# wangtong627/COR

Measured on AMD Instinct MI355X. Metric: query triplets/sec (forward + similarity + top-k), higher is better.
Workload: dtype bf16

## Files before the change

cor_amd/csrc/flash_attn.hip:

```cpp
#include <cstdlib>
#include <type_traits>

#include "common.h"

typedef short s16x4 __attribute__((ext_vector_type(4)));

namespace {

struct FlashArgs {
  const bf16_t* q; const bf16_t* k; const bf16_t* v; void* o;
  long q_sb, q_st, k_sb, k_st, v_sb, v_st, o_sb, o_st;
  int H, Tq, Tk;
  float scale_log2;
  float tbl_scale;
  const bf16_t* pad_row; const float* rel_h; const float* rel_w;
  int grid, S, nW, d3;
  int nqt;
  int rev;
};

constexpr int KT = 64;
constexpr int TILE_B = KT * 128;
constexpr int KV_BYTES = 4 * TILE_B;
constexpr int AUX_PER_WAVE = 8192;
constexpr float LOG2E = 1.4426950408889634f;

__device__ __forceinline__ int acc_row(int e, int h) { return (e & 3) + 8 * (e >> 2) + 4 * h; }

__device__ __forceinline__ float other_half(float x) {
  const unsigned u = __float_as_uint(x);
  const auto r = __builtin_amdgcn_permlane32_swap(u, u, false, false);
  return __uint_as_float((threadIdx.x & 32) ? r[0] : r[1]);
}

typedef float f32x2_t __attribute__((ext_vector_type(2)));
typedef __bf16 bf16x2_t __attribute__((ext_vector_type(2)));
__device__ __forceinline__ uint32_t pk2(float a, float b) {
  const f32x2_t v = {a, b};
  return __builtin_bit_cast(uint32_t, __builtin_convertvector(v, bf16x2_t));
}
__device__ __forceinline__ uint4 pack8(float f0, float f1, float f2, float f3, float f4, float f5, float f6, float f7) {
  uint4 u;
  u.x = pk2(f0, f1); u.y = pk2(f2, f3); u.z = pk2(f4, f5); u.w = pk2(f6, f7);
  return u;
}

__device__ __forceinline__ float sum2_bf16(uint32_t pair, float acc) {
  return __builtin_amdgcn_fdot2_f32_bf16(__builtin_bit_cast(bf16x2_t, pair), __builtin_bit_cast(bf16x2_t, 0x3f803f80u), acc, false);
}
__device__ __forceinline__ float max3f_(float a, float b, float c) { return fmaxf(fmaxf(a, b), c); }

__device__ __forceinline__ uint4 table_frag(const float* tbl, int j, int c, int h) {
  const float* p = tbl + (long)j * 64 + 16 * c + 8 * h;
  const f32x4 a = *(const f32x4*)p, b = *(const f32x4*)(p + 4);
  return pack8(a[0], a[1], a[2], a[3], b[0], b[1], b[2], b[3]);
}

template <typename TO, int HD, typename OFF>
__device__ __forceinline__ void store_o_rows(const f32x16 (&o)[(HD + 31) / 32], float inv, char* stg, TO* out, int lane, OFF&& off) {
  constexpr int DB = (HD + 31) / 32;
  const int r = lane & 31, h = lane >> 5;
  if constexpr (sizeof(TO) == 2) {
    constexpr int SR = HD * 2 + 16, NCHO = HD * 2 / 16;
#pragma unroll
    for (int db = 0; db < DB; ++db)
#pragma unroll
      for (int g = 0; g < 4; ++g) {
        if (db * 32 + 8 * g + 8 <= HD) {
          uint2 u;
          u.x = pk2(o[db][4 * g] * inv, o[db][4 * g + 1] * inv); u.y = pk2(o[db][4 * g + 2] * inv, o[db][4 * g + 3] * inv);
          *(uint2*)(stg + r * SR + (db * 32 + 8 * g + 4 * h) * 2) = u;
        }
      }
    __builtin_amdgcn_fence(__ATOMIC_ACQ_REL, "wavefront");
#pragma unroll
    for (int i = 0; i < (32 * NCHO + 63) / 64; ++i) {
      const int idx = lane + 64 * i, j = idx / NCHO, ch = idx - j * NCHO;
      if (idx < 32 * NCHO) {
        const uint4 v = *(const uint4*)(stg + j * SR + ch * 16);
        const long e = off(j);
        if (e >= 0) *(uint4*)(out + e + ch * 8) = v;
      }
    }
  } else {
#pragma unroll
    for (int db = 0; db < DB; ++db) {
#pragma unroll
      for (int g = 0; g < 4; ++g) {
        if (db * 32 + 8 * g + 8 <= HD) {
          const f32x4 v4 = {o[db][4 * g] * inv, o[db][4 * g + 1] * inv, o[db][4 * g + 2] * inv, o[db][4 * g + 3] * inv};
          *(f32x4*)(stg + r * 144 + (8 * g + 4 * h) * 4) = v4;
        }
      }
      __builtin_amdgcn_fence(__ATOMIC_ACQ_REL, "wavefront");
#pragma unroll
      for (int i = 0; i < 4; ++i) {
        const int j = (lane >> 3) + 8 * i, ch = lane & 7;
        const f32x4 v = *(const f32x4*)(stg + j * 144 + ch * 16);
        const long e = off(j);
        if (e >= 0 && db * 32 + 4 * ch + 4 <= HD) *(f32x4*)(out + e + db * 32 + ch * 4) = v;
      }
      __builtin_amdgcn_fence(__ATOMIC_ACQ_REL, "wavefront");
    }
  }
}

template <int HD>
__device__ __forceinline__ uint4 table_frag_hd(const float* tbl, int j, int c, int h) {
  if (16 * c + 8 * h + 8 > HD) return make_uint4(0, 0, 0, 0);
  const float* p = tbl + (long)j * HD + 16 * c + 8 * h;
  const f32x4 a = *(const f32x4*)p, b = *(const f32x4*)(p + 4);
  return pack8(a[0], a[1], a[2], a[3], b[0], b[1], b[2], b[3]);
}

template <int MODE, typename TO, int HD = 64>
__global__ void __launch_bounds__(256, 2) flash_fwd(const FlashArgs a) {
  extern __shared__ __attribute__((aligned(16))) char smem[];
  constexpr int KS = (HD + 15) / 16, DB = (HD + 31) / 32, NCH = HD * 2 / 16, NCHP = 2 * KS;
  constexpr int ROWB = HD == 64 ? 128 : 208, TILEB = KT * ROWB, KVB = 4 * TILEB;
  constexpr int NP = (KT * NCHP + 255) / 256;
  const int tid = threadIdx.x, lane = tid & 63, wave = tid >> 6;
  const int r = lane & 31, h = lane >> 5;
  const int wi0_ = xcd_remap(blockIdx.x, gridDim.x);
  const int wi_ = a.rev ? (int)gridDim.x - 1 - wi0_ : wi0_;
  const int qt_ = wi_ % a.nqt, hb_ = wi_ / a.nqt;
  const int head = hb_ % a.H, bz = hb_ / a.H;
  const int S = a.S;

  int b = bz, wy = 0, wx = 0;
  if (MODE == 2) { const int nw2 = a.nW * a.nW; b = bz / nw2; const int wi = bz - b * nw2; wy = wi / a.nW; wx = wi - wy * a.nW; }
  const int g2 = a.grid * a.grid;

  auto kv_src = [&](int kidx, const bf16_t*& kp, const bf16_t*& vp) {
    if (MODE == 0) {
      kp = a.k + bz * a.k_sb + (long)kidx * a.k_st + head * HD;
      vp = a.v + bz * a.v_sb + (long)kidx * a.v_st + head * HD;
    } else {
      long row; bool ok = true;
      if (MODE == 1) row = (long)b * g2 + kidx;
      else {
        const int ky = kidx / S, kx = kidx - ky * S, y = wy * S + ky, x = wx * S + kx;
        ok = y < a.grid && x < a.grid;
        row = (long)b * g2 + (long)y * a.grid + x;
      }
      const bf16_t* base = ok ? a.q + row * a.d3 : a.pad_row;
      kp = base + a.H * HD + head * HD;
      vp = base + 2 * a.H * HD + head * HD;
    }
  };

  int tq = qt_ * 128 + wave * 32 + r;
  bool qvalid = tq < a.Tq;
  tq = min(tq, a.Tq - 1);
  const int qh = MODE == 0 ? 0 : tq / S, qw = MODE == 0 ? 0 : tq - (tq / S) * S;
  const bf16_t* qp;
  long orow = 0;
  if (MODE == 0) qp = a.q + bz * a.q_sb + (long)tq * a.q_st + head * HD;
  else if (MODE == 1) { orow = (long)b * g2 + tq; qp = a.q + orow * a.d3 + head * HD; }
  else {
    const int y = wy * S + qh, x = wx * S + qw;
    const bool ok = y < a.grid && x < a.grid;
    qvalid = qvalid && ok;
    orow = (long)b * g2 + (long)min(y, a.grid - 1) * a.grid + min(x, a.grid - 1);
    qp = ok ? a.q + orow * a.d3 + head * HD : a.pad_row + head * HD;
  }
  uint4 qf[KS];
#pragma unroll
  for (int c = 0; c < KS; ++c) qf[c] = (16 * c + 8 * h + 8 <= HD) ? *(const uint4*)(qp + 16 * c + 8 * h) : make_uint4(0, 0, 0, 0);

  constexpr int TSTRIDE = MODE == 2 ? 56 : KT;
  int st_row[NP], st_ch[NP], st_k[NP], st_v[NP];
// ... 720 lines not shown
    if (t + 3 < nt) vsrc += tile_bytes;
    if (!(DBG & 1) && (DBG & 512)) { dma_tile(kd, vk0p, vk1p, ksrc_t); dma_tile(vd, vv0p, vv1p, vsrc_t); }
    const char *Vs = Vring + ((t + 3) & 3) * TILE_B, *Ks = Kring + ((t + 1) & 3) * TILE_B;
    const float rh0 = aux[t * 64 + r], rh1 = aux[t * 64 + 32 + r];
    u32x4 vf[8], kf[8];
    if (DBG & 4) { Vs = Vring; Ks = Kring; }
#pragma unroll
    for (int i = 0; i < 8; ++i) {
      const int kb = i >> 2, ks = (i >> 1) & 1, db = i & 1;
      if ((DBG & 4) && t > 0) { vf[i] = u32x4{(unsigned)t, (unsigned)i, 3u, 4u}; continue; }
      const char* vb = Vs + (kb * 32 + ks * 16) * 128 + v_trd[db];
      const s16x4 v0 = __builtin_amdgcn_ds_read_tr16_b64_v4i16((__attribute__((address_space(3))) s16x4*)(vb));
      const s16x4 v1 = __builtin_amdgcn_ds_read_tr16_b64_v4i16((__attribute__((address_space(3))) s16x4*)(vb + 8 * 128));
      vf[i] = __builtin_bit_cast(u32x4, __builtin_shufflevector(v0, v1, 0, 1, 2, 3, 4, 5, 6, 7));
    }
#pragma unroll
    for (int i = 0; i < 8; ++i) {
      if ((DBG & 4) && t > 0) { kf[i] = u32x4{(unsigned)t, (unsigned)i, 1u, 2u}; continue; }
      kf[i] = *(const u32x4*)(Ks + (i >> 2) * 32 * 128 + kch[i & 3]);
    }
    __builtin_amdgcn_sched_barrier(0);

    auto pv = [&](int n) __attribute__((always_inline)) {
      const int qb = n >> 3, kb = (n >> 2) & 1, ks = (n >> 1) & 1, db = n & 1;
      if (DBG & 32) { asm volatile("" : "+a"(o[qb][db]) : "a"(vf[kb * 4 + ks * 2 + db]), "v"(pf[qb][kb][ks])); return; }
      asm volatile("v_mfma_f32_32x32x16_bf16 %0, %1, %2, %0" : "+a"(o[qb][db]) : "a"(vf[kb * 4 + ks * 2 + db]), "v"(pf[qb][kb][ks]));
    };
    auto qk = [&](int g, int c) __attribute__((always_inline)) {
      const int qb = g >> 1, kb = g & 1;
      if (DBG & 64) { asm volatile("" : "+v"(s[qb][kb]) : "a"(kf[kb * 4 + c]), "a"(qf[qb][c]), "v"(wreg[qb][kb])); return; }
      if (c == 0) asm volatile("v_mfma_f32_32x32x16_bf16 %0, %1, %2, %3" : "=&v"(s[qb][kb]) : "a"(kf[kb * 4 + c]), "a"(qf[qb][c]), "v"(wreg[qb][kb]));
      else asm volatile("v_mfma_f32_32x32x16_bf16 %0, %1, %2, %0" : "+v"(s[qb][kb]) : "a"(kf[kb * 4 + c]), "a"(qf[qb][c]));
    };
    float mloc[2];
#pragma unroll
    for (int qb = 0; qb < 2; ++qb) {
      float m4[4];
#pragma unroll
      for (int kb = 0; kb < 2; ++kb)
#pragma unroll
        for (int g = 0; g < 2; ++g) {
          const int e = 8 * g;
          const f32x16& x = s[qb][kb];
          if (DBG & 16) { m4[kb * 2 + g] = x[e]; continue; }
          const float t0 = max3f_(x[e], x[e + 1], x[e + 2]), t1 = max3f_(x[e + 3], x[e + 4], x[e + 5]);
          m4[kb * 2 + g] = max3f_(max3f_(t0, t1, x[e + 6]), x[e + 7], -INFINITY);
        }
      mloc[qb] = fmaxf(max3f_(m4[0], m4[1], m4[2]), m4[3]);
      __builtin_amdgcn_sched_barrier(0);
      pv(qb);
    }
    float msub[2], al0 = 1.f, al1 = 1.f;
    bool resc;
    {
      const float ml0 = fmaxf(mloc[0], other_half(mloc[0])) + rh0, ml1 = fmaxf(mloc[1], other_half(mloc[1])) + rh1;
      resc = __builtin_amdgcn_ballot_w64(ml0 > m[0] + 8.0f || ml1 > m[1] + 8.0f) != 0;
      if (resc) {
        const float mn0 = fmaxf(m[0], ml0), mn1 = fmaxf(m[1], ml1);
        al0 = __builtin_amdgcn_exp2f(m[0] - mn0); al1 = __builtin_amdgcn_exp2f(m[1] - mn1);
        m[0] = mn0; m[1] = mn1;
        lsum[0][0] *= al0; lsum[0][1] *= al0; lsum[1][0] *= al1; lsum[1][1] *= al1;
      }
      msub[0] = m[0] - rh0; msub[1] = m[1] - rh1;
    }
    __builtin_amdgcn_sched_barrier(0);
    float pe[4] = {0.f, 0.f, 0.f, 0.f};
#pragma unroll
    for (int c = 0; c <= 16; ++c) {
      float pn[4];
      uint32_t d0 = 0, d1 = 0;
      const int cp = c - 1, gp = cp >> 2, qbp = gp >> 1, kbp = gp & 1, k4 = cp & 3;
      if (c < 16) {
        const int g = c >> 2, qb = g >> 1, kb = g & 1, e0 = 4 * (c & 3);
#pragma unroll
        for (int i = 0; i < 2; ++i) pn[i] = (DBG & 8) ? s[qb][kb][e0 + i] - msub[qb] : (DBG & 256) ? __builtin_amdgcn_exp2f(s[qb][kb][e0 + i]) : __builtin_amdgcn_exp2f(s[qb][kb][e0 + i] - msub[qb]);
      }
      if (c > 0) { d0 = pk2(pe[0], pe[1]); if (!(DBG & 128)) lsum[qbp][k4 & 1] = sum2_bf16(d0, lsum[qbp][k4 & 1]); else if (c == 1) lsum[qbp][k4 & 1] += __uint_as_float(d0); }
      if (!(DBG & 1) && !(DBG & 512)) {
        if (c == 2) dma_tile(kd, vk0p, vk1p, ksrc_t);
        if (c == 10) dma_tile(vd, vv0p, vv1p, vsrc_t);
      }
      if (c < 4) pv(2 + 2 * c);
      else if (c < 8) pv(6 + c);
      else if (c < 10) pv(6 + c);
      else if (c < 12) qk(1, c - 8);
      else if (c < 16) qk(2, c - 12);
      __builtin_amdgcn_sched_barrier(0);
      if (c < 16) {
        const int g = c >> 2, qb = g >> 1, kb = g & 1, e0 = 4 * (c & 3);
#pragma unroll
        for (int i = 2; i < 4; ++i) pn[i] = (DBG & 8) ? s[qb][kb][e0 + i] - msub[qb] : (DBG & 256) ? __builtin_amdgcn_exp2f(s[qb][kb][e0 + i]) : __builtin_amdgcn_exp2f(s[qb][kb][e0 + i] - msub[qb]);
      }
      if (c > 0) {
        d1 = pk2(pe[2], pe[3]); if (!(DBG & 128)) lsum[qbp][k4 & 1] = sum2_bf16(d1, lsum[qbp][k4 & 1]);
        u32x4& dst = pf[qbp][kbp][k4 >> 1];
        if (k4 & 1) { dst[2] = d0; dst[3] = d1; } else { dst[0] = d0; dst[1] = d1; }
      }
      if (c < 4) pv(3 + 2 * c);
      else if (c < 8) qk(0, c - 4);
      else if (c < 10) qk(1, c - 8);
      else if (c == 16) { qk(3, 0); qk(3, 1); qk(3, 2); qk(3, 3); }
#pragma unroll
      for (int i = 0; i < 4; ++i) pe[i] = pn[i];
      __builtin_amdgcn_sched_barrier(0);
    }
    asm volatile("" :: "v"(lsum[0][0]), "v"(lsum[0][1]), "v"(lsum[1][0]), "v"(lsum[1][1]));
    if (resc) {
#pragma unroll
      for (int db = 0; db < 2; ++db)
#pragma unroll
        for (int e = 0; e < 16; ++e) {
          float x0 = o[0][db][e], x1 = o[1][db][e], t0, t1;
          asm volatile("v_accvgpr_read_b32 %2, %0\n\tv_accvgpr_read_b32 %3, %1\n\tv_mul_f32 %2, %2, %4\n\tv_mul_f32 %3, %3, %5\n\t"
                       "v_accvgpr_write_b32 %0, %2\n\tv_accvgpr_write_b32 %1, %3"
                       : "+a"(x0), "+a"(x1), "=&v"(t0), "=&v"(t1) : "v"(al0), "v"(al1));
          o[0][db][e] = x0; o[1][db][e] = x1;
        }
    }
    if (!(DBG & 2)) {
      asm volatile("s_waitcnt vmcnt(6)" ::: "memory");
      __syncthreads();
    }
  }
  {
    asm volatile("s_waitcnt vmcnt(0)" ::: "memory");
    const char* Vs = Vring + ((nt - 1) & 3) * TILE_B;
#pragma unroll
    for (int kb = 0; kb < 2; ++kb)
#pragma unroll
      for (int ks = 0; ks < 2; ++ks)
#pragma unroll
        for (int db = 0; db < 2; ++db) {
          const char* vb = Vs + (kb * 32 + ks * 16) * 128 + v_trd[db];
          const s16x4 v0 = __builtin_amdgcn_ds_read_tr16_b64_v4i16((__attribute__((address_space(3))) s16x4*)(vb));
          const s16x4 v1 = __builtin_amdgcn_ds_read_tr16_b64_v4i16((__attribute__((address_space(3))) s16x4*)(vb + 8 * 128));
          const u32x4 vfr = __builtin_bit_cast(u32x4, __builtin_shufflevector(v0, v1, 0, 1, 2, 3, 4, 5, 6, 7));
#pragma unroll
          for (int qb = 0; qb < 2; ++qb)
            asm volatile("v_mfma_f32_32x32x16_bf16 %0, %1, %2, %0" : "+a"(o[qb][db]) : "a"(vfr), "v"(pf[qb][kb][ks]));
        }
    asm volatile("s_nop 7\n\ts_nop 7\n\ts_nop 7\n\ts_nop 7" ::: "memory");
  }
#pragma unroll
  for (int qb = 0; qb < 2; ++qb) {
    const float l = lsum[qb][0] + lsum[qb][1];
    const float inv = 1.0f / (l + other_half(l));
    auto off = [&](int j) -> long { return ((long)b * g2 + qh * S + qb * 32 + j) * (long)(a.H * 64) + head * 64; };
    store_o_rows<TO, 64>(o[qb], inv, (char*)aux, (TO*)a.o, lane, off);
    __builtin_amdgcn_fence(__ATOMIC_ACQ_REL, "wavefront");
  }
}

constexpr int WIN_ROWS = 224, WIN_KV = WIN_ROWS * 128, WIN_T = 27 * 32 * 4, WIN_LDS = 2 * WIN_KV + 7 * WIN_T;

template <typename TO>
__global__ void __launch_bounds__(448, 4) win_attn(const FlashArgs a) {
  extern __shared__ __attribute__((aligned(16))) char smem[];
  const int tid = threadIdx.x, lane = tid & 63, wave = __builtin_amdgcn_readfirstlane(tid >> 6);
  const int r = lane & 31, h = lane >> 5;
  const int bid = a.rev ? (int)gridDim.x - 1 - (int)blockIdx.x : (int)blockIdx.x;
  const int head = bid % a.H, win = bid / a.H;
  const int nw2 = a.nW * a.nW, b = win / nw2, wi = win - b * nw2, wy = wi / a.nW, wx = wi - wy * a.nW;
  const int g2 = a.grid * a.grid;
  char* Kt = smem; char* Vt = smem + WIN_KV;
  float* T = (float*)(smem + 2 * WIN_KV + wave * WIN_T);

  {
    const unsigned lds0 = __builtin_amdgcn_readfirstlane((unsigned)(size_t)((__attribute__((address_space(3))) char*)smem));
    const int sl = lane & 7;
    long colp[2]; bool okx[2];
#pragma unroll
    for (int hf = 0; hf < 2; ++hf) {
      const int kw = min(8 * hf + (lane >> 3), 13), x = wx * 14 + kw;
      okx[hf] = x < a.grid;
      colp[hf] = ((long)b * g2 + x) * a.d3 + head * 64;
    }
#pragma unroll
    for (int i8 = 0; i8 < 8; ++i8) {
      const int i = wave * 8 + i8;
      const bool isv = i >= 28;
      const int ii = isv ? i - 28 : i, kh = ii >> 1, hf = ii & 1, y = wy * 14 + kh;
      const int chunk = isv ? (sl ^ (((lane >> 4) & 1) << 2)) : (sl ^ (4 * hf + (lane >> 4)));
      const long plane = (long)(isv ? 2 : 1) * a.H * 64 + chunk * 8;
      const bf16_t* src = (y < a.grid && okx[hf]) ? a.q + colp[hf] + (long)y * a.grid * a.d3 + plane : a.pad_row + head * 64 + plane;
      glds16(src, lds0 + (isv ? WIN_KV : 0) + ii * 1024);
    }
  }

  const int tq = min(wave * 32 + r, 195);
  const int qh = (tq * 4682) >> 16, qw = tq - 14 * qh;
  uint4 qf[4];
  {
    const int y = wy * 14 + qh, x = wx * 14 + qw;
    const bf16_t* qp = (y < a.grid && x < a.grid) ? a.q + ((long)b * g2 + (long)y * a.grid + x) * a.d3 + head * 64 : a.pad_row + head * 64;
#pragma unroll
    for (int c = 0; c < 4; ++c) qf[c] = *(const uint4*)(qp + 16 * c + 8 * h);
  }

  float colb[8];
  uint4 tf[2][4];
#pragma unroll
  for (int tbl = 0; tbl < 2; ++tbl)
#pragma unroll
    for (int c = 0; c < 4; ++c) tf[tbl][c] = table_frag(tbl == 0 ? a.rel_w : a.rel_h, min(r, 26), c, h);
#pragma unroll
  for (int tbl = 0; tbl < 2; ++tbl) {
    f32x16 acc;
#pragma unroll
    for (int e = 0; e < 16; ++e) acc[e] = 0.f;
#pragma unroll
    for (int c = 0; c < 4; ++c)
      acc = __builtin_amdgcn_mfma_f32_32x32x16_bf16(__builtin_bit_cast(bf16x8, tf[tbl][c]), __builtin_bit_cast(bf16x8, qf[c]), acc, 0, 0, 0);
#pragma unroll
    for (int e = 0; e < 16; ++e) {
      const int row = acc_row(e, h);
      if (row < 27) T[row * 32 + r] = acc[e] * a.tbl_scale;
    }
    __builtin_amdgcn_fence(__ATOMIC_ACQ_REL, "wavefront");
    if (tbl == 0) {
#pragma unroll
      for (int e8 = 0; e8 < 8; ++e8) {
        const int kw = (e8 & 3) + 8 * (e8 >> 2) + 4 * h;
        colb[e8] = kw < 14 ? T[(qw - min(kw, 13) + 13) * 32 + r] : -INFINITY;
      }
      __builtin_amdgcn_fence(__ATOMIC_ACQ_REL, "wavefront");
    }
  }

  if (a.scale_log2 != 1.0f) {
#pragma unroll
    for (int c = 0; c < 4; ++c) {
      uint32_t w[4] = {qf[c].x, qf[c].y, qf[c].z, qf[c].w};
#pragma unroll
      for (int i = 0; i < 4; ++i) w[i] = pk2(__uint_as_float(w[i] << 16) * a.scale_log2, __uint_as_float(w[i] & 0xffff0000u) * a.scale_log2);
      qf[c] = make_uint4(w[0], w[1], w[2], w[3]);
    }
  }

  asm volatile("s_waitcnt vmcnt(0)" ::: "memory");
  __syncthreads();

  const int sw = (r >> 1) & 7;
  const int k_rd = r * 128, v_tr = (4 * h + ((lane & 15) >> 2)) * 128 + (16 * ((lane >> 4) & 1) + 4 * (lane & 3)) * 2;
  const int v_trd[2] = {v_tr + ((lane >> 3) & 1) * 64, v_tr + (1 - ((lane >> 3) & 1)) * 64};
  const int t_rd = (qh + 13) * 32 + r;
  f32x16 o[2], lsum;
#pragma unroll
  for (int e = 0; e < 16; ++e) { o[0][e] = 0.f; o[1][e] = 0.f; lsum[e] = 0.f; }
  float m = 0.f;
  const uint4 ones = make_uint4(0x3F803F80u, 0x3F803F80u, 0x3F803F80u, 0x3F803F80u);
#pragma unroll
  for (int blk = 0; blk < 7; ++blk) {
    const char* Kb = Kt + blk * 32 * 128 + k_rd;
    uint4 kf[4];
#pragma unroll
    for (int c = 0; c < 4; ++c) kf[c] = *(const uint4*)(Kb + (((2 * c + h) ^ sw) << 4));
    const float rm0 = T[t_rd - 32 * (2 * blk)] - m, rm1 = T[t_rd - 32 * (2 * blk + 1)] - m;
    f32x16 s;
#pragma unroll
    for (int e = 0; e < 16; ++e) s[e] = colb[e & 7] + (e < 8 ? rm0 : rm1);
#pragma unroll
    for (int c = 0; c < 4; ++c)
      s = __builtin_amdgcn_mfma_f32_32x32x16_bf16(__builtin_bit_cast(bf16x8, kf[c]), __builtin_bit_cast(bf16x8, qf[c]), s, 0, 0, 0);
    float mloc = max3f_(max3f_(s[0], s[1], s[2]), max3f_(s[3], s[4], s[5]), max3f_(s[6], s[7], s[8]));
    mloc = fmaxf(max3f_(mloc, max3f_(s[9], s[10], s[11]), max3f_(s[12], s[13], s[14])), s[15]);
    mloc = fmaxf(mloc, other_half(mloc));
    if (blk == 0 || __builtin_amdgcn_ballot_w64(mloc > 8.0f) != 0) {
      const float d = blk == 0 ? mloc : fmaxf(mloc, 0.f);
      const float alpha = __builtin_amdgcn_exp2f(-d);
      m += d;
#pragma unroll
      for (int e = 0; e < 16; ++e) s[e] -= d;
      if (blk != 0) {
        lsum[1] *= alpha; lsum[2] *= alpha;
#pragma unroll
        for (int e = 0; e < 16; ++e) { o[0][e] *= alpha; o[1][e] *= alpha; }
      }
    }
    uint4 pf[2];
    {
      f32x16 p;
#pragma unroll
      for (int e = 0; e < 16; ++e) p[e] = __builtin_amdgcn_exp2f(s[e]);
      pf[0] = pack8(p[0], p[1], p[2], p[3], p[4], p[5], p[6], p[7]);
      pf[1] = pack8(p[8], p[9], p[10], p[11], p[12], p[13], p[14], p[15]);
      lsum[1] = sum2_bf16(pf[0].y, sum2_bf16(pf[0].x, lsum[1])); lsum[2] = sum2_bf16(pf[0].w, sum2_bf16(pf[0].z, lsum[2]));
      lsum[1] = sum2_bf16(pf[1].y, sum2_bf16(pf[1].x, lsum[1])); lsum[2] = sum2_bf16(pf[1].w, sum2_bf16(pf[1].z, lsum[2]));
    }
#pragma unroll
    for (int ks = 0; ks < 2; ++ks) {
#pragma unroll
      for (int db = 0; db < 2; ++db) {
        const char* vb = Vt + (blk * 32 + ks * 16) * 128 + v_trd[db];
        const s16x4 v0 = __builtin_amdgcn_ds_read_tr16_b64_v4i16((__attribute__((address_space(3))) s16x4*)(vb));
        const s16x4 v1 = __builtin_amdgcn_ds_read_tr16_b64_v4i16((__attribute__((address_space(3))) s16x4*)(vb + 8 * 128));
        const uint2 u0 = __builtin_bit_cast(uint2, v0), u1 = __builtin_bit_cast(uint2, v1);
        const uint4 vfr = make_uint4(u0.x, u0.y, u1.x, u1.y);
        o[db] = __builtin_amdgcn_mfma_f32_32x32x16_bf16(__builtin_bit_cast(bf16x8, vfr), __builtin_bit_cast(bf16x8, pf[ks]), o[db], 0, 0, 0);
      }
    }
  }

  const float lhalf = lsum[1] + lsum[2];
  const float inv = 1.0f / (lhalf + other_half(lhalf));
  char* stg = (char*)T;
  TO* out = (TO*)a.o;
  auto off = [&](int jq) -> long {
    const int tj = wave * 32 + jq;
    if (tj >= 196) return -1;
    const int jh = (tj * 4682) >> 16, y = wy * 14 + jh, x = wx * 14 + (tj - 14 * jh);
    if (y >= a.grid || x >= a.grid) return -1;
    return ((long)b * g2 + (long)y * a.grid + x) * (long)(a.H * 64) + head * 64;
  };
  const long e0 = off(lane >> 2), e1 = off((lane >> 2) + 16);
  const int rd0 = (lane >> 2) * 80 + (lane & 3) * 16;
  __builtin_amdgcn_fence(__ATOMIC_ACQ_REL, "wavefront");
  if constexpr (sizeof(TO) == 2) {
#pragma unroll
    for (int db = 0; db < 2; ++db) {
#pragma unroll
      for (int g = 0; g < 4; ++g) {
        uint2 u;
        u.x = pk2(o[db][4 * g] * inv, o[db][4 * g + 1] * inv); u.y = pk2(o[db][4 * g + 2] * inv, o[db][4 * g + 3] * inv);
        *(uint2*)(stg + r * 80 + (8 * g + 4 * h) * 2) = u;
      }
      __builtin_amdgcn_fence(__ATOMIC_ACQ_REL, "wavefront");
      const uint4 v0 = *(const uint4*)(stg + rd0), v1 = *(const uint4*)(stg + rd0 + 16 * 80);
      if (e0 >= 0) *(uint4*)(out + e0 + db * 32 + (lane & 3) * 8) = v0;
      if (e1 >= 0) *(uint4*)(out + e1 + db * 32 + (lane & 3) * 8) = v1;
      __builtin_amdgcn_fence(__ATOMIC_ACQ_REL, "wavefront");
    }
  } else {
#pragma unroll
    for (int qd = 0; qd < 4; ++qd) {
      const int db = qd >> 1, g0 = 2 * (qd & 1);
#pragma unroll
      for (int gg = 0; gg < 2; ++gg) {
        const int g = g0 + gg;
        const f32x4 v4 = {o[db][4 * g] * inv, o[db][4 * g + 1] * inv, o[db][4 * g + 2] * inv, o[db][4 * g + 3] * inv};
        *(f32x4*)(stg + r * 80 + (8 * gg + 4 * h) * 4) = v4;
      }
      __builtin_amdgcn_fence(__ATOMIC_ACQ_REL, "wavefront");
      const f32x4 v0 = *(const f32x4*)(stg + rd0), v1 = *(const f32x4*)(stg + rd0 + 16 * 80);
      if (e0 >= 0) *(f32x4*)(out + e0 + qd * 16 + (lane & 3) * 4) = v0;
      if (e1 >= 0) *(f32x4*)(out + e1 + qd * 16 + (lane & 3) * 4) = v1;
      __builtin_amdgcn_fence(__ATOMIC_ACQ_REL, "wavefront");
    }
  }
}

template <typename TO>
int launch_win(const FlashArgs& a, int nwin, hipStream_t s) {
  static DevOnce once;
  cor_max_dyn_lds((const void*)win_attn<TO>, WIN_LDS, once);
  hipLaunchKernelGGL((win_attn<TO>), dim3(nwin * a.H), dim3(448), WIN_LDS, s, a);
  COR_CHECK_LAUNCH();
  return 0;
}

template <typename TO, bool STAMP = false, bool CB = false>
int launch_global_pipe(const FlashArgs& a, int nb, hipStream_t s) {
  const size_t lds = 6 * TILE_B + 4 * AUX_PER_WAVE;
  static DevOnce once;
  cor_max_dyn_lds((const void*)flash_global_pipe<TO, STAMP, CB>, (int)lds, once);
  FlashArgs b = a;
  b.nqt = cdiv(a.Tq, 128);
  hipLaunchKernelGGL((flash_global_pipe<TO, STAMP, CB>), dim3(b.nqt * a.H * nb), dim3(256), lds, s, b);
  COR_CHECK_LAUNCH();
  return 0;
}

template <typename TO, int DBG = 0>
int launch_global_w64(const FlashArgs& a, int nb, hipStream_t s) {
  const size_t lds = 8 * TILE_B + 4 * 64 * 64 * 4;
  static DevOnce once;
  cor_max_dyn_lds((const void*)flash_global_w64<TO, DBG>, (int)lds, once);
  FlashArgs b = a;
  b.nqt = a.Tq / 256;
  hipLaunchKernelGGL((flash_global_w64<TO, DBG>), dim3(b.nqt * a.H * nb), dim3(256), lds, s, b);
  COR_CHECK_LAUNCH();
  return 0;
}

template <int MODE, typename TO, int HD = 64>
int launch(const FlashArgs& a, int nb, hipStream_t s) {
  constexpr int ROWB = HD == 64 ? 128 : 208;
  const size_t lds = 4 * KT * ROWB + (MODE == 0 ? 0 : 4 * AUX_PER_WAVE);
  static DevOnce once;
  cor_max_dyn_lds((const void*)flash_fwd<MODE, TO, HD>, (int)lds, once);
  FlashArgs b = a;
  b.nqt = cdiv(a.Tq, 128);
  hipLaunchKernelGGL((flash_fwd<MODE, TO, HD>), dim3(b.nqt * a.H * nb), dim3(256), lds, s, b);
  COR_CHECK_LAUNCH();
  return 0;
}
template <int MODE, int HD>
int launch_t(const FlashArgs& a, int nb, int out_dtype, hipStream_t s) {
  if (out_dtype == COR_BF16) return launch<MODE, bf16_t, HD>(a, nb, s);
  if (out_dtype == COR_F32) return launch<MODE, float, HD>(a, nb, s);
  return COR_ENOSUPPORT;
}

}

int cor_flash_plain_bf16(const void* q, long q_sb, long q_st, const void* k, long k_sb, long k_st, const void* v, long v_sb, long v_st,
                         void* out, long o_sb, long o_st, int out_dtype, int B, int H, int Tq, int Tk, int hd, float scale, hipStream_t s) {
  if ((q_st | k_st | v_st | q_sb | k_sb | v_sb) & 7) return COR_ENOSUPPORT;
  if (((uintptr_t)q | (uintptr_t)k | (uintptr_t)v | (uintptr_t)out) & 15) return COR_ENOSUPPORT;
  if ((o_st | o_sb) & 7) return COR_ENOSUPPORT;
  FlashArgs a{};
  a.q = (const bf16_t*)q; a.k = (const bf16_t*)k; a.v = (const bf16_t*)v; a.o = out;
  a.q_sb = q_sb; a.q_st = q_st; a.k_sb = k_sb; a.k_st = k_st; a.v_sb = v_sb; a.v_st = v_st; a.o_sb = o_sb; a.o_st = o_st;
  a.H = H; a.Tq = Tq; a.Tk = Tk; a.scale_log2 = scale * LOG2E; a.tbl_scale = LOG2E; a.S = 1; a.grid = 1; a.nW = 1;
  if (hd == 64) return launch_t<0, 64>(a, B, out_dtype, s);
  if (hd == 72) return launch_t<0, 72>(a, B, out_dtype, s);
  if (hd == 80) return launch_t<0, 80>(a, B, out_dtype, s);
  return COR_ENOSUPPORT;
}

int cor_flash_sam_bf16(const void* qkv, void* out, int out_dtype, const void* pad_row, const float* rel_h, const float* rel_w, int B,
                       int H, int hd, int grid, int window, float q_prescale, int variant, hipStream_t s) {
  if (hd != 64 && hd != 80) return COR_ENOSUPPORT;
  const int rev = (variant & COR_ORDER_REVERSE) ? 1 : 0;
  variant &= ~COR_ORDER_REVERSE;
#ifdef COR_PROBES
  if (variant != 0 && variant != 1 && variant != 2 && variant != 4 && variant != 9 && !(variant >= 16 && variant < 4096)) return COR_EINVAL;
#else
  if (variant != 0 && variant != 1 && variant != 2 && variant != 4) return COR_EINVAL;
#endif
  if (((uintptr_t)qkv & 15) || ((uintptr_t)out & 15) || ((uintptr_t)rel_h & 15) || ((uintptr_t)rel_w & 15)) return COR_ENOSUPPORT;
  FlashArgs a{};
  a.q = (const bf16_t*)qkv; a.o = out; a.H = H; a.rev = rev;
  a.scale_log2 = LOG2E / sqrtf((float)hd) / q_prescale; a.tbl_scale = LOG2E / q_prescale;
  if (hd == 64 && fabsf(a.scale_log2 - 1.0f) < 1e-6f) { a.scale_log2 = 1.0f; a.tbl_scale = 8.0f; }
  a.pad_row = (const bf16_t*)pad_row; a.rel_h = rel_h; a.rel_w = rel_w; a.grid = grid; a.d3 = 3 * H * hd;
  if (window == 0) {
    if (grid != 64) return COR_ENOSUPPORT;
    a.S = 64; a.Tq = a.Tk = grid * grid; a.nW = 1;
#ifdef COR_PROBES
    if (const char* e = getenv("COR_ATTN_TK")) a.Tk = atoi(e);
#endif
    if (hd == 80) return launch_t<1, 80>(a, B, out_dtype, s);
#ifdef COR_PROBES
    if (variant >= 16 && out_dtype == COR_BF16 && a.scale_log2 == 1.0f) {
      switch (variant - 16) {
        case 1: return launch_global_w64<bf16_t, 1>(a, B, s);
        case 2: return launch_global_w64<bf16_t, 2>(a, B, s);
        case 3: return launch_global_w64<bf16_t, 3>(a, B, s);
        case 4: return launch_global_w64<bf16_t, 4>(a, B, s);
        case 8: return launch_global_w64<bf16_t, 8>(a, B, s);
        case 16: return launch_global_w64<bf16_t, 16>(a, B, s);
        case 32: return launch_global_w64<bf16_t, 32>(a, B, s);
        case 64: return launch_global_w64<bf16_t, 64>(a, B, s);
        case 96: return launch_global_w64<bf16_t, 96>(a, B, s);
        case 7: return launch_global_w64<bf16_t, 7>(a, B, s);
        case 127: return launch_global_w64<bf16_t, 127>(a, B, s);
        case 128: return launch_global_w64<bf16_t, 128>(a, B, s);
        case 256: return launch_global_w64<bf16_t, 256>(a, B, s);
        case 384: return launch_global_w64<bf16_t, 384>(a, B, s);
        case 512: return launch_global_w64<bf16_t, 512>(a, B, s);
        default: return COR_EINVAL;
      }
    }
    if (variant == 9) {
      if (out_dtype == COR_BF16) return launch_global_pipe<bf16_t, true>(a, B, s);
      if (out_dtype == COR_F32) return launch_global_pipe<float, true>(a, B, s);
    }
#endif
    if (variant == 4 && a.scale_log2 == 1.0f) {
      if (out_dtype == COR_BF16) return launch_global_w64<bf16_t>(a, B, s);
      if (out_dtype == COR_F32) return launch_global_w64<float>(a, B, s);
    }
    if (variant == 0 && a.scale_log2 == 1.0f) {
      if (out_dtype == COR_BF16) return launch_global_pipe<bf16_t, false, true>(a, B, s);
      if (out_dtype == COR_F32) return launch_global_pipe<float, false, true>(a, B, s);
    }
    if (variant == 0 || variant == 2 || variant == 4) {
      if (out_dtype == COR_BF16) return launch_global_pipe<bf16_t>(a, B, s);
      if (out_dtype == COR_F32) return launch_global_pipe<float>(a, B, s);
    }
    if (out_dtype == COR_BF16) return launch<1, bf16_t>(a, B, s);
    if (out_dtype == COR_F32) return launch<1, float>(a, B, s);
    return COR_ENOSUPPORT;
  }
  if (window != 14 || ((uintptr_t)pad_row & 15)) return COR_ENOSUPPORT;
  a.S = 14; a.Tq = a.Tk = 196; a.nW = (grid + 13) / 14;
  if (hd == 80) return launch_t<2, 80>(a, B * a.nW * a.nW, out_dtype, s);
  if (variant != 1) {
    if (out_dtype == COR_BF16) return launch_win<bf16_t>(a, B * a.nW * a.nW, s);
    if (out_dtype == COR_F32) return launch_win<float>(a, B * a.nW * a.nW, s);
    return COR_ENOSUPPORT;
  }
  if (out_dtype == COR_BF16) return launch<2, bf16_t>(a, B * a.nW * a.nW, s);
  if (out_dtype == COR_F32) return launch<2, float>(a, B * a.nW * a.nW, s);
  return COR_ENOSUPPORT;
}
```

Baseline: 765.0.

## Add persistent double-buffered windowed attention kernel overlapping next-unit K/V loads

Windowed attention now defaults to a persistent kernel that loops over (window, head) units with a grid sized to CUs × occupancy × rounds. While computing the current unit it prefetches the next unit's K/V into a second LDS buffer and loads its Q, hiding global load latency behind the compute. The original one-block-per-unit kernel stays available as variant 8, and timestamp probes are added behind the probe build. The trade-off is launch bounds of 1 block per CU with twice the K/V LDS, which lowers occupancy and may reduce latency hiding across blocks.

```diff
diff --git a/cor_amd/csrc/flash_attn.hip b/cor_amd/csrc/flash_attn.hip
--- a/cor_amd/csrc/flash_attn.hip
+++ b/cor_amd/csrc/flash_attn.hip
@@ -17,6 +17,7 @@
   int grid, S, nW, d3;
   int nqt;
   int rev;
+  unsigned long long* stamps;
 };
 
 constexpr int KT = 64;
@@ -1043,57 +1044,61 @@
 }
 
 constexpr int WIN_ROWS = 224, WIN_KV = WIN_ROWS * 128, WIN_T = 27 * 32 * 4, WIN_LDS = 2 * WIN_KV + 7 * WIN_T;
-
-template <typename TO>
-__global__ void __launch_bounds__(448, 4) win_attn(const FlashArgs a) {
-  extern __shared__ __attribute__((aligned(16))) char smem[];
-  const int tid = threadIdx.x, lane = tid & 63, wave = __builtin_amdgcn_readfirstlane(tid >> 6);
-  const int r = lane & 31, h = lane >> 5;
-  const int bid = a.rev ? (int)gridDim.x - 1 - (int)blockIdx.x : (int)blockIdx.x;
-  const int head = bid % a.H, win = bid / a.H;
-  const int nw2 = a.nW * a.nW, b = win / nw2, wi = win - b * nw2, wy = wi / a.nW, wx = wi - wy * a.nW;
+constexpr int WINP_LDS = 4 * WIN_KV + 7 * WIN_T;
+#ifndef WINP_ROUNDS
+#define WINP_ROUNDS 2
+#endif
+
+struct WinUnit { int b, wy, wx, head; };
+__device__ __forceinline__ WinUnit win_unit(const FlashArgs& a, int bid) {
+  WinUnit u;
+  u.head = bid % a.H;
+  const int win = bid / a.H, nw2 = a.nW * a.nW;
+  u.b = win / nw2;
+  const int wi = win - u.b * nw2;
+  u.wy = wi / a.nW; u.wx = wi - u.wy * a.nW;
+  return u;
+}
+
+__device__ __forceinline__ void win_kv_dma(const FlashArgs& a, const WinUnit& u, int wave, int lane, unsigned lds0) {
   const int g2 = a.grid * a.grid;
-  char* Kt = smem; char* Vt = smem + WIN_KV;
-  float* T = (float*)(smem + 2 * WIN_KV + wave * WIN_T);
-
-  {
-    const unsigned lds0 = __builtin_amdgcn_readfirstlane((unsigned)(size_t)((__attribute__((address_space(3))) char*)smem));
-    const int sl = lane & 7;
-    long colp[2]; bool okx[2];
-#pragma unroll
-    for (int hf = 0; hf < 2; ++hf) {
-      const int kw = min(8 * hf + (lane >> 3), 13), x = wx * 14 + kw;
-      okx[hf] = x < a.grid;
-      colp[hf] = ((long)b * g2 + x) * a.d3 + head * 64;
-    }
-#pragma unroll
-    for (int i8 = 0; i8 < 8; ++i8) {
-      const int i = wave * 8 + i8;
-      const bool isv = i >= 28;
-      const int ii = isv ? i - 28 : i, kh = ii >> 1, hf = ii & 1, y = wy * 14 + kh;
-      const int chunk = isv ? (sl ^ (((lane >> 4) & 1) << 2)) : (sl ^ (4 * hf + (lane >> 4)));
-      const long plane = (long)(isv ? 2 : 1) * a.H * 64 + chunk * 8;
-      const bf16_t* src = (y < a.grid && okx[hf]) ? a.q + colp[hf] + (long)y * a.grid * a.d3 + plane : a.pad_row + head * 64 + plane;
-      glds16(src, lds0 + (isv ? WIN_KV : 0) + ii * 1024);
-    }
-  }
-
-  const int tq = min(wave * 32 + r, 195);
-  const int qh = (tq * 4682) >> 16, qw = tq - 14 * qh;
-  uint4 qf[4];
-  {
-    const int y = wy * 14 + qh, x = wx * 14 + qw;
-    const bf16_t* qp = (y < a.grid && x < a.grid) ? a.q + ((long)b * g2 + (long)y * a.grid + x) * a.d3 + head * 64 : a.pad_row + head * 64;
-#pragma unroll
-    for (int c = 0; c < 4; ++c) qf[c] = *(const uint4*)(qp + 16 * c + 8 * h);
-  }
-
-  float colb[8];
-  uint4 tf[2][4];
+  const int sl = lane & 7;
+  long colp[2]; bool okx[2];
+#pragma unroll
+  for (int hf = 0; hf < 2; ++hf) {
+    const int kw = min(8 * hf + (lane >> 3), 13), x = u.wx * 14 + kw;
+    okx[hf] = x < a.grid;
+    colp[hf] = ((long)u.b * g2 + x) * a.d3 + u.head * 64;
+  }
+#pragma unroll
+  for (int i8 = 0; i8 < 8; ++i8) {
+    const int i = wave * 8 + i8;
+    const bool isv = i >= 28;
+    const int ii = isv ? i - 28 : i, kh = ii >> 1, hf = ii & 1, y = u.wy * 14 + kh;
+    const int chunk = isv ? (sl ^ (((lane >> 4) & 1) << 2)) : (sl ^ (4 * hf + (lane >> 4)));
+    const long plane = (long)(isv ? 2 : 1) * a.H * 64 + chunk * 8;
+    const bf16_t* src = (y < a.grid && okx[hf]) ? a.q + colp[hf] + (long)y * a.grid * a.d3 + plane : a.pad_row + u.head * 64 + plane;
+    glds16(src, lds0 + (isv ? WIN_KV : 0) + ii * 1024);
+  }
+}
+
+__device__ __forceinline__ void win_q_load(const FlashArgs& a, const WinUnit& u, int qh, int qw, int h, uint4 (&qf)[4]) {
+  const int y = u.wy * 14 + qh, x = u.wx * 14 + qw;
+  const bf16_t* qp = (y < a.grid && x < a.grid) ? a.q + ((long)u.b * a.grid * a.grid + (long)y * a.grid + x) * a.d3 + u.head * 64
+                                                : a.pad_row + u.head * 64;
+#pragma unroll
+  for (int c = 0; c < 4; ++c) qf[c] = *(const uint4*)(qp + 16 * c + 8 * h);
+}
+
+__device__ __forceinline__ void win_table_frags(const FlashArgs& a, int r, int h, uint4 (&tf)[2][4]) {
 #pragma unroll
   for (int tbl = 0; tbl < 2; ++tbl)
 #pragma unroll
     for (int c = 0; c < 4; ++c) tf[tbl][c] = table_frag(tbl == 0 ? a.rel_w : a.rel_h, min(r, 26), c, h);
+}
+
+__device__ __forceinline__ void win_tables(const FlashArgs& a, const uint4 (&qf)[4], const uint4 (&tf)[2][4], float* T, int r, int h,
+                                           int qw, float (&colb)[8]) {
 #pragma unroll
   for (int tbl = 0; tbl < 2; ++tbl) {
     f32x16 acc;
@@ -1117,7 +1122,9 @@
       __builtin_amdgcn_fence(__ATOMIC_ACQ_REL, "wavefront");
     }
   }
-
+}
+
+__device__ __forceinline__ void win_prescale(const FlashArgs& a, uint4 (&qf)[4]) {
   if (a.scale_log2 != 1.0f) {
 #pragma unroll
     for (int c = 0; c < 4; ++c) {
@@ -1127,19 +1134,19 @@
       qf[c] = make_uint4(w[0], w[1], w[2], w[3]);
     }
   }
-
-  asm volatile("s_waitcnt vmcnt(0)" ::: "memory");
-  __syncthreads();
-
+}
+
+__device__ __forceinline__ void win_keys(const char* Kt, const float* T, const uint4 (&qf)[4], const float (&colb)[8], int lane, int qh,
+                                         f32x16 (&o)[2], f32x16& lsum) {
+  const char* Vt = Kt + WIN_KV;
+  const int r = lane & 31, h = lane >> 5;
   const int sw = (r >> 1) & 7;
   const int k_rd = r * 128, v_tr = (4 * h + ((lane & 15) >> 2)) * 128 + (16 * ((lane >> 4) & 1) + 4 * (lane & 3)) * 2;
   const int v_trd[2] = {v_tr + ((lane >> 3) & 1) * 64, v_tr + (1 - ((lane >> 3) & 1)) * 64};
   const int t_rd = (qh + 13) * 32 + r;
-  f32x16 o[2], lsum;
 #pragma unroll
   for (int e = 0; e < 16; ++e) { o[0][e] = 0.f; o[1][e] = 0.f; lsum[e] = 0.f; }
   float m = 0.f;
-  const uint4 ones = make_uint4(0x3F803F80u, 0x3F803F80u, 0x3F803F80u, 0x3F803F80u);
 #pragma unroll
   for (int blk = 0; blk < 7; ++blk) {
     const char* Kb = Kt + blk * 32 * 128 + k_rd;
@@ -1191,17 +1198,22 @@
       }
     }
   }
-
+}
+
+template <typename TO>
+__device__ __forceinline__ void win_store(const FlashArgs& a, const WinUnit& u, int wave, int lane, const f32x16 (&o)[2], const f32x16& lsum,
+                                          char* stg) {
+  const int r = lane & 31, h = lane >> 5;
+  const int g2 = a.grid * a.grid;
   const float lhalf = lsum[1] + lsum[2];
   const float inv = 1.0f / (lhalf + other_half(lhalf));
-  char* stg = (char*)T;
   TO* out = (TO*)a.o;
   auto off = [&](int jq) -> long {
     const int tj = wave * 32 + jq;
     if (tj >= 196) return -1;
-    const int jh = (tj * 4682) >> 16, y = wy * 14 + jh, x = wx * 14 + (tj - 14 * jh);
+    const int jh = (tj * 4682) >> 16, y = u.wy * 14 + jh, x = u.wx * 14 + (tj - 14 * jh);
     if (y >= a.grid || x >= a.grid) return -1;
-    return ((long)b * g2 + (long)y * a.grid + x) * (long)(a.H * 64) + head * 64;
+    return ((long)u.b * g2 + (long)y * a.grid + x) * (long)(a.H * 64) + u.head * 64;
   };
   const long e0 = off(lane >> 2), e1 = off((lane >> 2) + 16);
   const int rd0 = (lane >> 2) * 80 + (lane & 3) * 16;
@@ -1211,9 +1223,9 @@
     for (int db = 0; db < 2; ++db) {
 #pragma unroll
       for (int g = 0; g < 4; ++g) {
-        uint2 u;
-        u.x = pk2(o[db][4 * g] * inv, o[db][4 * g + 1] * inv); u.y = pk2(o[db][4 * g + 2] * inv, o[db][4 * g + 3] * inv);
-        *(uint2*)(stg + r * 80 + (8 * g + 4 * h) * 2) = u;
+        uint2 w;
+        w.x = pk2(o[db][4 * g] * inv, o[db][4 * g + 1] * inv); w.y = pk2(o[db][4 * g + 2] * inv, o[db][4 * g + 3] * inv);
+        *(uint2*)(stg + r * 80 + (8 * g + 4 * h) * 2) = w;
       }
       __builtin_amdgcn_fence(__ATOMIC_ACQ_REL, "wavefront");
       const uint4 v0 = *(const uint4*)(stg + rd0), v1 = *(const uint4*)(stg + rd0 + 16 * 80);
@@ -1240,11 +1252,139 @@
   }
 }
 
-template <typename TO>
+__device__ __forceinline__ unsigned long long win_clock() {
+  __builtin_amdgcn_sched_barrier(0);
+  const unsigned long long t = __builtin_readcyclecounter();
+  __builtin_amdgcn_sched_barrier(0);
+  return t;
+}
+__device__ __forceinline__ void win_stamps_out(const FlashArgs& a, int wave, int lane, const unsigned long long (&ts)[8]) {
+  if (lane == 0) {
+#pragma unroll
+    for (int i = 0; i < 8; ++i) a.stamps[((long)blockIdx.x * 7 + wave) * 8 + i] = ts[i];
+  }
+}
+
+template <typename TO, bool STAMP = false>
+__global__ void __launch_bounds__(448, 4) win_attn(const FlashArgs a) {
+  extern __shared__ __attribute__((aligned(16))) char smem[];
+  const int tid = threadIdx.x, lane = tid & 63, wave = __builtin_amdgcn_readfirstlane(tid >> 6);
+  const int r = lane & 31, h = lane >> 5;
+  const WinUnit u = win_unit(a, a.rev ? (int)gridDim.x - 1 - (int)blockIdx.x : (int)blockIdx.x);
+  float* T = (float*)(smem + 2 * WIN_KV + wave * WIN_T);
+  unsigned long long ts[8] = {0, 0, 0, 0, 0, 0, 0, 0}, t0 = 0, t1;
+  if (STAMP) t0 = win_clock();
+
+  win_kv_dma(a, u, wave, lane, __builtin_amdgcn_readfirstlane((unsigned)(size_t)((__attribute__((address_space(3))) char*)smem)));
+  const int tq = min(wave * 32 + r, 195);
+  const int qh = (tq * 4682) >> 16, qw = tq - 14 * qh;
+  uint4 qf[4];
+  win_q_load(a, u, qh, qw, h, qf);
+  uint4 tf[2][4];
+  win_table_frags(a, r, h, tf);
+  float colb[8];
+  win_tables(a, qf, tf, T, r, h, qw, colb);
+  win_prescale(a, qf);
+  if (STAMP) { t1 = win_clock(); ts[0] += t1 - t0; t0 = t1; }
+
+  asm volatile("s_waitcnt vmcnt(0)" ::: "memory");
+  __syncthreads();
+  if (STAMP) { t1 = win_clock(); ts[1] += t1 - t0; t0 = t1; }
+
+  f32x16 o[2], lsum;
+  win_keys(smem, T, qf, colb, lane, qh, o, lsum);
+  if (STAMP) { t1 = win_clock(); ts[2] += t1 - t0; t0 = t1; }
+  win_store<TO>(a, u, wave, lane, o, lsum, (char*)T);
+  if (STAMP) { t1 = win_clock(); ts[3] += t1 - t0; win_stamps_out(a, wave, lane, ts); }
+}
+
+template <typename TO, bool STAMP = false>
+__global__ void __launch_bounds__(448, 1) win_attn_pp(const FlashArgs a) {
+  extern __shared__ __attribute__((aligned(16))) char smem[];
+  const int tid = threadIdx.x, lane = tid & 63, wave = __builtin_amdgcn_readfirstlane(tid >> 6);
+  const int r = lane & 31, h = lane >> 5;
+  const int units = a.nqt;
+  const unsigned lds0 = __builtin_amdgcn_readfirstlane((unsigned)(size_t)((__attribute__((address_space(3))) char*)smem));
+  float* T = (float*)(smem + 4 * WIN_KV + wave * WIN_T);
+  unsigned long long ts[8] = {0, 0, 0, 0, 0, 0, 0, 0}, t0 = 0, t1;
+  if (STAMP) t0 = win_clock();
+
+  int ui = blockIdx.x;
+  WinUnit u = win_unit(a, a.rev ? units - 1 - ui : ui);
+  win_kv_dma(a, u, wave, lane, lds0);
+  const int tq = min(wave * 32 + r, 195);
+  const int qh = (tq * 4682) >> 16, qw = tq - 14 * qh;
+  uint4 qf[4];
+  win_q_load(a, u, qh, qw, h, qf);
+  uint4 tf[2][4];
+  win_table_frags(a, r, h, tf);
+  float colb[8];
+  win_tables(a, qf, tf, T, r, h, qw, colb);
+  win_prescale(a, qf);
+  asm volatile("s_waitcnt vmcnt(0)" ::: "memory");
+  __syncthreads();
+  if (STAMP) { t1 = win_clock(); ts[5] += t1 - t0; t0 = t1; }
+
+  for (int it = 0;; ++it) {
+    const int un = ui + (int)gridDim.x;
+    const bool more = un < units;
+    WinUnit c = u;
+    uint4 qn[4];
+    if (more) {
+      c = win_unit(a, a.rev ? units - 1 - un : un);
+      win_kv_dma(a, c, wave, lane, lds0 + ((it + 1) & 1) * (2 * WIN_KV));
+      win_q_load(a, c, qh, qw, h, qn);
+    }
+    if (STAMP) { t1 = win_clock(); ts[0] += t1 - t0; t0 = t1; }
+    f32x16 o[2], lsum;
+    win_keys(smem + (it & 1) * (2 * WIN_KV), T, qf, colb, lane, qh, o, lsum);
+    if (STAMP) { t1 = win_clock(); ts[1] += t1 - t0; t0 = t1; }
+    win_store<TO>(a, u, wave, lane, o, lsum, (char*)T);
+    if (STAMP) { t1 = win_clock(); ts[2] += t1 - t0; t0 = t1; }
+    if (!more) break;
+    ui = un; u = c;
+#pragma unroll
+    for (int k = 0; k < 4; ++k) qf[k] = qn[k];
+    win_tables(a, qf, tf, T, r, h, qw, colb);
+    win_prescale(a, qf);
+    if (STAMP) { t1 = win_clock(); ts[3] += t1 - t0; t0 = t1; }
+    asm volatile("s_waitcnt vmcnt(0)" ::: "memory");
+    __syncthreads();
+    if (STAMP) { t1 = win_clock(); ts[4] += t1 - t0; t0 = t1; }
+  }
+  if (STAMP) win_stamps_out(a, wave, lane, ts);
+}
+
+template <typename TO, bool STAMP = false>
 int launch_win(const FlashArgs& a, int nwin, hipStream_t s) {
   static DevOnce once;
-  cor_max_dyn_lds((const void*)win_attn<TO>, WIN_LDS, once);
-  hipLaunchKernelGGL((win_attn<TO>), dim3(nwin * a.H), dim3(448), WIN_LDS, s, a);
+  cor_max_dyn_lds((const void*)win_attn<TO, STAMP>, WIN_LDS, once);
+  hipLaunchKernelGGL((win_attn<TO, STAMP>), dim3(nwin * a.H), dim3(448), WIN_LDS, s, a);
+  COR_CHECK_LAUNCH();
+  return 0;
+}
+
+template <typename TO, bool STAMP = false>
+int launch_win_pp(const FlashArgs& a, int nwin, hipStream_t s) {
+  static DevOnce once;
+  static std::atomic<int> per_cu[COR_MAX_DEVICES] = {};
+  const void* fn = (const void*)win_attn_pp<TO, STAMP>;
+  cor_max_dyn_lds(fn, WINP_LDS, once);
+  const int d = cor_cur_device();
+  int occ = per_cu[d].load(std::memory_order_acquire);
+  if (occ == 0) {
+    if (hipOccupancyMaxActiveBlocksPerMultiprocessor(&occ, fn, 448, WINP_LDS) != hipSuccess || occ < 1) occ = 1;
+    per_cu[d].store(occ, std::memory_order_release);
+  }
+  FlashArgs b = a;
+  b.nqt = nwin * a.H;
+  int rounds = WINP_ROUNDS;
+#ifdef COR_PROBES
+  if (const char* e = getenv("COR_WIN_ROUNDS")) rounds = atoi(e) > 0 ? atoi(e) : rounds;
+#endif
+  const long slots = (long)cor_device_cus() * occ * rounds;
+  const int grid = (int)(slots < b.nqt ? slots : b.nqt);
+  hipLaunchKernelGGL((win_attn_pp<TO, STAMP>), dim3(grid), dim3(448), WINP_LDS, s, b);
   COR_CHECK_LAUNCH();
   return 0;
 }
@@ -1315,9 +1455,10 @@
   const int rev = (variant & COR_ORDER_REVERSE) ? 1 : 0;
   variant &= ~COR_ORDER_REVERSE;
 #ifdef COR_PROBES
-  if (variant != 0 && variant != 1 && variant != 2 && variant != 4 && variant != 9 && !(variant >= 16 && variant < 4096)) return COR_EINVAL;
+  if (variant != 0 && variant != 1 && variant != 2 && variant != 4 && variant != 8 && variant != 9 && variant != 10 && !(variant >= 16 && variant < 4096))
+    return COR_EINVAL;
 #else
-  if (variant != 0 && variant != 1 && variant != 2 && variant != 4) return COR_EINVAL;
+  if (variant != 0 && variant != 1 && variant != 2 && variant != 4 && variant != 8) return COR_EINVAL;
 #endif
   if (((uintptr_t)qkv & 15) || ((uintptr_t)out & 15) || ((uintptr_t)rel_h & 15) || ((uintptr_t)rel_w & 15)) return COR_ENOSUPPORT;
   FlashArgs a{};
@@ -1328,6 +1469,10 @@
   if (window == 0) {
     if (grid != 64) return COR_ENOSUPPORT;
     a.S = 64; a.Tq = a.Tk = grid * grid; a.nW = 1;
+    if (variant == 8) variant = 0;
+#ifdef COR_PROBES
+    if (variant == 10) return COR_EINVAL;
+#endif
 #ifdef COR_PROBES
     if (const char* e = getenv("COR_ATTN_TK")) a.Tk = atoi(e);
 #endif
@@ -1377,9 +1522,23 @@
   if (window != 14 || ((uintptr_t)pad_row & 15)) return COR_ENOSUPPORT;
   a.S = 14; a.Tq = a.Tk = 196; a.nW = (grid + 13) / 14;
   if (hd == 80) return launch_t<2, 80>(a, B * a.nW * a.nW, out_dtype, s);
+  const int nwin = B * a.nW * a.nW;
+#ifdef COR_PROBES
+  if (variant == 9 || variant == 10) {
+    a.stamps = (unsigned long long*)((char*)out + (long)B * grid * grid * H * 64 * (out_dtype == COR_F32 ? 4 : 2));
+    if (out_dtype == COR_BF16) return variant == 9 ? launch_win<bf16_t, true>(a, nwin, s) : launch_win_pp<bf16_t, true>(a, nwin, s);
+    if (out_dtype == COR_F32) return variant == 9 ? launch_win<float, true>(a, nwin, s) : launch_win_pp<float, true>(a, nwin, s);
+    return COR_ENOSUPPORT;
+  }
+#endif
+  if (variant == 8) {
+    if (out_dtype == COR_BF16) return launch_win<bf16_t>(a, nwin, s);
+    if (out_dtype == COR_F32) return launch_win<float>(a, nwin, s);
+    return COR_ENOSUPPORT;
+  }
   if (variant != 1) {
-    if (out_dtype == COR_BF16) return launch_win<bf16_t>(a, B * a.nW * a.nW, s);
-    if (out_dtype == COR_F32) return launch_win<float>(a, B * a.nW * a.nW, s);
+    if (out_dtype == COR_BF16) return launch_win_pp<bf16_t>(a, nwin, s);
+    if (out_dtype == COR_F32) return launch_win_pp<float>(a, nwin, s);
     return COR_ENOSUPPORT;
   }
   if (out_dtype == COR_BF16) return launch<2, bf16_t>(a, B * a.nW * a.nW, s);
```

Result: no change. 767.4, median of 6 (+0.3%).
